# dimfeld/perceive

Hardware: AMD Instinct MI355X
Metric: vectors scanned/sec (exact cosine top-10, 384-d f32, batch=64) (higher is better)
Workload: dtype f32

## Files before the change

### perceive_amd/csrc/scan.h

```cpp
#pragma once
#include <hip/hip_runtime.h>
#include <stdint.h>

#include "../../include/perceive_hip.h"

namespace pcv {

constexpr int kBlockRows = 32;
constexpr int kMaxK = PCV_MAX_RESULTS;
constexpr int kSeedPartRows = 256;
constexpr int kSeedParts = 64;
constexpr int kMaxWaveQueries = 4;
constexpr int kHot = 256;
constexpr int kMfmaQueries = 256;
constexpr int kScale8Stride = 1;

struct SegDesc {
    const float4* blk;
    const float* scale;
    const int64_t* ids;
    int64_t id0;
    int64_t pos0;
    uint32_t nrows;
    uint32_t nblocks;
// ... 54 lines not shown

struct ScanParams {
    const SegDesc* seg;
    int nseg;
    uint32_t total_blocks;
    int D;
    int D4;
    int B;
    int k;
    int metric;
    uint32_t tile_rows;
    const CeilRec* ceil;
    const float* queries;
    float* qf32;
    uint16_t* qbf16;
    int8_t* q8;
    float* q8c;
    float* qraw;
    float* margin;
    float* margin32;
    uint32_t* tau;
    uint32_t* tau_c;
    uint32_t* slots;
    uint32_t* cand_cnt;
    uint64_t* cand;
    float* cand_s;
    pcv_hit_dev* out;
    pcv_hit_dev* out_host;
    uint32_t* cnt_host;
    uint32_t* coarse_host;
    pcv_hit_dev* flag_rec;
    uint32_t cand_cap;
    uint32_t seed_blocks;
    uint32_t seed_shift;
    uint32_t flags;
    unsigned long long* stamps;
    float eps16, eps32;
    float max_norm;
    uint32_t* spec;
    int spec_rank;
    float spec_gap;
    float spec_spread;
    float* spec_base_host;
    float* spec_top_host;
    float* kth_host;
    const RangeRec* range;
    pcv_hit_dev* range_out;
    uint32_t* range_cnt;
    uint32_t range_runs;
    uint32_t range_keep;
};
constexpr uint32_t kSpecFailed = 0xffffffffu;

struct DistinctRec {
    uint32_t kept, examined, flags, pad;
    double last_score;
    int64_t last_pos;
};
constexpr uint32_t kDistinctFull = 1u, kDistinctEnd = 2u;
struct DistinctArgs {
    DistinctRec* rec;
    DistinctRec* rec_host;
    pcv_hit_dev* kept;
    double* kept_norm;
    int32_t* similar;
    int num_results;
    double threshold;
};

struct GroupedArgs {
    DistinctRec* rec;
    DistinctRec* rec_host;
    pcv_hit_dev* kept;
    int64_t* kept_group;
// ... 29 lines not shown
    uint32_t u = (k & 0x80000000u) ? (k & 0x7fffffffu) : ~k;
    return __builtin_bit_cast(float, u);
}
constexpr uint32_t kKeyNegInf = 0x007fffffu;
__host__ __device__ static inline uint64_t f64_key(double d) {
    uint64_t u = __builtin_bit_cast(uint64_t, d);
    return (u >> 63) ? ~u : (u | 0x8000000000000000ull);
}
__host__ __device__ static inline double key_f64(uint64_t k) {
    uint64_t u = (k >> 63) ? (k & 0x7fffffffffffffffull) : ~k;
    return __builtin_bit_cast(double, u);
}

__host__ __device__ static inline float reported_score(int metric, int D, double c) {
    if (metric == PCV_METRIC_DOT) {
        const double d = 1.0 - c / (double)D;
        return (float)(d > 0.0 ? d : 0.0);
    }
    return (float)c;
}

void launch_upload(hipStream_t st, const void* src_pinned, void* dst, size_t bytes);
void launch_prep_seed(hipStream_t st, const ScanParams& p, const ScanParams* dp, const SegDesc& seg0);
void launch_scan_wave(hipStream_t st, const ScanParams& p, const ScanParams* dp, int num_cus);
void launch_scan_mfma(hipStream_t st, const ScanParams& p, const ScanParams* dp, int num_cus);
int mfma_pass_queries(int Dp);
uint32_t mfma_tile_rows(int B);
void launch_scan_mfma8(hipStream_t st, const ScanParams& p, const ScanParams* dp, int num_cus);
int mfma8_pass_queries(int Dp);
bool mfma8_six_pass(int B, int Dp, uint32_t flags, int nseg);
void launch_rescore_select(hipStream_t st, const ScanParams& p, const ScanParams* dp);
void launch_range_thresholds(hipStream_t st, const ScanParams& p, const ScanParams* dp);
void launch_range_select(hipStream_t st, const ScanParams& p, const ScanParams* dp);
void launch_distinct_select(hipStream_t st, const ScanParams& p, const ScanParams* dp, const DistinctArgs& a);
void launch_diverse_collect(hipStream_t st, const ScanParams& p, const ScanParams* dp, const DiverseArgs& a);
void launch_diverse_select(hipStream_t st, int B, int D, int D4, int metric, const DiverseArgs& a);
void launch_grouped_select(hipStream_t st, const ScanParams& p, const ScanParams* dp, const GroupedArgs& a);
void launch_reset_scan_state(hipStream_t st, uint32_t* tau, uint32_t* slots, uint32_t* cand_cnt);
void launch_merge(hipStream_t st, const pcv_hit_dev* lists, int n_shards, int B, int k, pcv_hit_dev* out,
                  int flagged = 0);
void launch_similarity_matrix(hipStream_t st, const float* a, int B, const float* m, int64_t N, int D, int cosine,
                              float* out);

}
```

### perceive_amd/csrc/scan_kernels.hip

```cpp
#include <algorithm>
#include <cassert>
#include <cstdlib>
#include <numeric>
#include <type_traits>

#include "common.h"
#include "device_access.h"
#include "scan.h"

namespace pcv {
namespace {

struct SegCursor {
    int si = -1;
    uint32_t begin = 0, end = 0;
    const float4* blk = nullptr;
    const float* scale = nullptr;
    const uint4* blk16 = nullptr;
    const uint4* blk8 = nullptr;
    const float* scale8 = nullptr;
    const uint4* mid16 = nullptr;
    const float* scale16 = nullptr;
    const uint4* blk6 = nullptr;
    const float4* scale6 = nullptr;
// ... 116 lines not shown
            }
            active = false;
        }
    }
}

__device__ __noinline__ void emit_hit(const ScanParams& p, int q, int seg, uint32_t row, float s,
                                      bool feeds_slots) {
    const int cc = ceil_class(p, q, s);
    if (cc == 2) return;
    feeds_slots = feeds_slots && cc == 0;
    uint32_t idx = g_atomic_add(&p.cand_cnt[q * kHot], 1u);
    if (idx < p.cand_cap) {
        gst(&p.cand[(size_t)q * p.cand_cap + idx], ((uint64_t)(uint32_t)seg << 32) | row);
        gst(&p.cand_s[(size_t)q * p.cand_cap + idx], s);
    }
    if (feeds_slots && isfinite(s)) offer_slot(p, q, s);
}


__global__ __launch_bounds__(256) void reset_scan_state_kernel(uint32_t* __restrict__ tau, uint32_t* __restrict__ slots,
                                                               uint32_t* __restrict__ cand_cnt) {
    const int t = blockIdx.x * 256 + threadIdx.x;
    if (t < kMfmaQueries * kMaxK) slots[t] = kKeyNegInf;
    if (t < kMfmaQueries) {
        tau[t * kHot] = kKeyNegInf;
        tau[kMfmaQueries * kHot + t] = kKeyNegInf;
        cand_cnt[t * kHot] = 0;
        cand_cnt[t * kHot + 32] = 0;
        cand_cnt[t * kHot + 33] = 0;
        cand_cnt[t * kHot + 34] = 0;
        cand_cnt[t * kHot + 35] = 0;
    }
}

__device__ __forceinline__ bool is_seed_block(const ScanParams& p, int si, uint32_t lb) {
    return si == 0 && (lb & ((1u << p.seed_shift) - 1u)) == 0 && (lb >> p.seed_shift) < p.seed_blocks;
}

__device__ __forceinline__ uint32_t seed_threshold_key(const ScanParams& p, int q, int sub ) {
    uint32_t mn = 0xffffffffu;
    if (q < p.B)
        for (int j = sub; j < p.k; j += 4) mn = min(mn, ld_relaxed(&p.slots[(size_t)q * kMaxK + j]));
    mn = min(mn, (uint32_t)__shfl_xor(mn, 1));
    mn = min(mn, (uint32_t)__shfl_xor(mn, 2));
    return q < p.B ? mn : kKeyNegInf;
}
// ... 100 lines not shown
#pragma unroll
        for (int j = 0; j < 16; ++j)
#pragma unroll
            for (int g = 0; g < QG; ++g) {
                const float4 qv = *(const float4*)&sq[g * Dp + (f0 + j) * 4];
                acc[g] = fmaf(qv.x, v[j].x, acc[g]);
                acc[g] = fmaf(qv.y, v[j].y, acc[g]);
                acc[g] = fmaf(qv.z, v[j].z, acc[g]);
                acc[g] = fmaf(qv.w, v[j].w, acc[g]);
            }
    }
    {
        const uint32_t grp = sr % (uint32_t)p.k;
#pragma unroll
        for (int g = 0; g < QG; ++g) {
            const float s = acc[g] * sc;
            if (sc != 0.0f && isfinite(s) && (q0 + g >= p.B || ceil_class(p, q0 + g, s) == 0)) atomicMax(&gmax[g * kMaxK + grp], f32_key(s));
        }
    }
    __syncthreads();
    for (int i = tid; i < QG * p.k; i += 256) {
        const int g = i / p.k, j = i - g * p.k, q = q0 + g;
        const uint32_t key = gmax[g * kMaxK + j];
        if (q < p.B && key != kKeyNegInf) g_atomic_max(&p.slots[(size_t)q * kMaxK + j], key);
    }
}

__global__ __launch_bounds__(256) void prep_seed_mfma_kernel(const ScanParams* __restrict__ pp, const float4* __restrict__ seg0_blk,
                                                             const float* __restrict__ seg0_scale, uint32_t nseed) {
    const ScanParams& p = *pp;
    extern __shared__ __attribute__((aligned(16))) float smem[];
    const int Dp = p.D4 * 4, D = p.D, LD = Dp + 4;
    float* sq = smem;
    uint32_t* gmax = (uint32_t*)(smem + 32 * LD);
    const int part = blockIdx.x, q0 = blockIdx.y * 32, tid = threadIdx.x, lane = tid & 63;
    const int wave = __builtin_amdgcn_readfirstlane(tid >> 6);
    const int r = lane & 31, h = lane >> 5;
    const bool writer = part == 0;
    const uint32_t sb = part * 4 + wave;
    const uint32_t lb = sb << p.seed_shift;
    const bool active = sb < p.seed_blocks && lb * 32u < nseed;
    const int P = p.D4 >> 1;
    const float4* base = seg0_blk + (size_t)(active ? lb : 0) * p.D4 * 32 + h * 32 + r;
    float4 va[16], vb[16];
    auto load16 = [&](float4 (&v)[16], int m0) {
#pragma unroll
        for (int j = 0; j < 16; ++j) v[j] = (active && m0 + j < P) ? gld4(base + (size_t)(m0 + j) * 64) : make_float4(0, 0, 0, 0);
// ... 41 lines not shown
            }
        }
        if (writer && have && sub == 0) {
            float unit = 1.0f;
            if (p.metric == PCV_METRIC_DOT) unit = (float)sqrt(sum) * p.max_norm * 1.0001f;
            gst(&p.margin[q], (p.eps16 + p.eps32) * unit);
            gst(&p.margin32[q], 2.0f * p.eps32 * unit);
        }
    }
    if (writer && blockIdx.y == 0) {
        uint16_t* z = p.qbf16 + (size_t)p.B * Dp;
        const int nz = ((int)p.tile_rows > p.B) ? ((int)p.tile_rows - p.B) * Dp : 0;
        for (int i = tid; i < nz; i += 256) gst(&z[i], (uint16_t)0);
        if (tid == 0 && p.flag_rec) {
            pcv_hit_dev f;
            f.score = 0.0;
            f.pos = 0;
            f.id = 0;
            *p.flag_rec = f;
        }
    }
    __syncthreads();

    f32x16 acc;
#pragma unroll
    for (int i = 0; i < 16; ++i) acc[i] = 0.0f;
    const float* qrow = sq + r * LD + h * 4;
    auto mma16 = [&](const float4 (&v)[16], int m0) {
#pragma unroll
        for (int j = 0; j < 16; ++j) {
            if (m0 + j < P) {
                const float4 qv = *(const float4*)&qrow[(m0 + j) * 8];
                acc = __builtin_amdgcn_mfma_f32_32x32x2f32(v[j].x, qv.x, acc, 0, 0, 0);
                acc = __builtin_amdgcn_mfma_f32_32x32x2f32(v[j].y, qv.y, acc, 0, 0, 0);
                acc = __builtin_amdgcn_mfma_f32_32x32x2f32(v[j].z, qv.z, acc, 0, 0, 0);
                acc = __builtin_amdgcn_mfma_f32_32x32x2f32(v[j].w, qv.w, acc, 0, 0, 0);
            }
        }
    };
    for (int m0 = 0; m0 < P; m0 += 32) {
        if (m0 + 16 < P) load16(vb, m0 + 16);
        __builtin_amdgcn_sched_barrier(0);
        mma16(va, m0);
        if (m0 + 32 < P) load16(va, m0 + 32);
        __builtin_amdgcn_sched_barrier(0);
        if (m0 + 16 < P) mma16(vb, m0 + 16);
    }
    if (active) {
        float sc[16];
#pragma unroll
        for (int i = 0; i < 16; ++i) {
            const uint32_t row = lb * 32 + (i & 3) + 8 * (i >> 2) + 4 * h;
            sc[i] = row < nseed ? gld(&seg0_scale[row]) : 0.0f;
        }
        const float clo = (p.ceil && q0 + r < p.B) ? gld(&p.ceil[q0 + r].lo) : __builtin_inff();
#pragma unroll
        for (int i = 0; i < 16; ++i) {
            const float s = acc[i] * sc[i];
            const uint32_t sr = sb * 32 + (i & 3) + 8 * (i >> 2) + 4 * h;
            if (sc[i] != 0.0f && isfinite(s) && s < clo) atomicMax(&gmax[r * p.k + sr % (uint32_t)p.k], f32_key(s));
        }
    }
    __syncthreads();
    for (int i = tid; i < 32 * p.k; i += 256) {
        const int g = i / p.k, j = i - g * p.k, q = q0 + g;
        const uint32_t key = gmax[i];
        if (q < p.B && key != kKeyNegInf) g_atomic_max(&p.slots[(size_t)q * kMaxK + j], key);
    }
}

struct BlockCursor {
    uint32_t gb;
    SegCursor sc;
    uint32_t lb;
    __amdgpu_buffer_rsrc_t rows;
    int ch;
};

template <int NB, bool NTL>
__global__ __launch_bounds__(256) void scan_wave_kernel(const ScanParams* __restrict__ pp) {
    const ScanParams& p = *pp;
    extern __shared__ __attribute__((aligned(16))) float sq[];
    const int Dp = p.D4 * 4;
    for (int i = threadIdx.x; i < NB * Dp; i += 256) sq[i] = gld(&p.qf32[i]);
    __syncthreads();
    const int lane = threadIdx.x & 63;
    const uint32_t wave = __builtin_amdgcn_readfirstlane(threadIdx.x >> 6);
    const int r = lane & 31, h = lane >> 5;
    float mrg[NB];
    uint32_t tau0[NB];
// ... 370 lines not shown
        for (int off = 32; off > 0; off >>= 1) {
            guess = max(guess, (uint32_t)__shfl_xor(guess, off));
            med = max(med, (uint32_t)__shfl_xor(med, off));
            top = max(top, (uint32_t)__shfl_xor(top, off));
        }
        if (learned && med != kKeyNegInf) {
            const float fm = key_f32(med), ft = key_f32(top);
            const float g = fminf(fm + p.spec_gap, ft + (ft - fm));
            const bool alike = fabsf((ft - fm) - p.spec_spread) <= 0.5f * p.spec_spread;
            if (alike && isfinite(g)) guess = max(guess, f32_key(g));
        }
        if (lane == 0 && guess != kKeyNegInf) {
            g_atomic_max(&p.tau[q * kHot], guess);
            g_atomic_max(&p.tau_c[q], guess);
        }
    }
    if (lane == 0 && have && p.spec_base_host) {
        p.spec_base_host[q] = med != kKeyNegInf ? key_f32(med) : __builtin_nanf("");
        p.spec_top_host[q] = top != kKeyNegInf ? key_f32(top) : __builtin_nanf("");
    }
    if (lane == 0) p.spec[q] = guess;
}

__global__ __launch_bounds__(256) void set_guess_kernel(const ScanParams* __restrict__ pp) {
    const ScanParams& p = *pp;
    const int q = blockIdx.x * 4 + (threadIdx.x >> 6);
    set_guess(p, q, threadIdx.x & 63, q < p.B);
}

__global__ __launch_bounds__(256) void quantize_queries_kernel(const ScanParams* __restrict__ pp) {
    const ScanParams& p = *pp;
    const int lane = threadIdx.x & 63;
    const int q = blockIdx.x * 4 + (threadIdx.x >> 6);
    const int Dp = p.D4 * 4, Dp8 = (Dp + 127) & ~127;
    const bool have = q < p.B;
    const float* src = p.qf32 + (size_t)q * Dp;
    float x[16];
    float mx = 0.0f, l1 = 0.0f;
#pragma unroll
    for (int j = 0; j < 16; ++j) {
        const int i = lane + 64 * j;
        x[j] = (have && i < Dp) ? gld(&src[i]) : 0.0f;
    }
#pragma unroll
    for (int j = 0; j < 16; ++j) {
        mx = fmaxf(mx, fabsf(x[j]));
        l1 += fabsf(x[j]);
    }
#pragma unroll
    for (int off = 32; off > 0; off >>= 1) {
        mx = fmaxf(mx, __shfl_xor(mx, off));
        l1 += __shfl_xor(l1, off);
    }
    const float s_q = (mx > 0.0f && mx < __builtin_inff() && l1 < __builtin_inff()) ? 127.0f / mx : 0.0f;
    int8_t* row = p.q8 + (size_t)q * Dp8;
    double n2 = 0.0, e2 = 0.0;
    int qs = 0, qa = 0;
#pragma unroll
    for (int j = 0; j < 16; ++j) {
        const int i = lane + 64 * j;
        const int qi = max(-127, min(127, (int)rintf((s_q != 0.0f ? x[j] : 0.0f) * s_q)));
        if (i < Dp8) row[i] = (int8_t)qi;
        const double e = s_q != 0.0f ? (double)x[j] - (double)qi / (double)s_q : 0.0;
        n2 += (double)x[j] * (double)x[j];
        e2 += e * e;
        qs += qi;
        qa += abs(qi);
    }
#pragma unroll
    for (int off = 32; off > 0; off >>= 1) {
        n2 += __shfl_xor(n2, off);
        e2 += __shfl_xor(e2, off);
        qs += __shfl_xor(qs, off);
        qa += __shfl_xor(qa, off);
    }
    if (lane == 0) {
        p.q8c[4 * q] = s_q;
        p.q8c[4 * q + 1] = 0.5002f * l1 * s_q + 0.2501f * (float)Dp8 + 4.0f;
        p.q8c[4 * q + 2] = l1;
        const bool live = have && s_q != 0.0f;
        const double W = 126.5 * (double)qs, M = 252.0 * (double)qa + fabs(W);
        const float up = 1.0f + 0x1p-19f;
        const float wn = (float)(-W + M * 0x1p-20);
        p.q8c[4 * kMfmaQueries + 4 * q] = live ? (float)(sqrt(n2) * (double)s_q) * up : 0.0f;
        p.q8c[4 * kMfmaQueries + 4 * q + 1] = live ? (float)(sqrt(e2) * (double)s_q) * up : 0.0f;
        p.q8c[4 * kMfmaQueries + 4 * q + 2] = live ? wn + fabsf(wn) * 0x1p-22f : 0.0f;
    }
    set_guess(p, q, lane, have);
}

template <int FROM, int TO, class F>
__device__ __forceinline__ bool static_for_until(F&& f) {
    if constexpr (FROM < TO) {
        if (f(std::integral_constant<int, FROM>{})) return true;
        return static_for_until<FROM + 1, TO>(f);
    } else {
        return false;
    }
}

constexpr uint32_t kRing = 2048;
constexpr int kRingSegBits = 18;
struct SurvRing {
    uint32_t lo[kRing], hi[kRing];
    int acc[kRing];
    float sblk[kRing];
    uint32_t tail, head, done, pad;
};
__device__ __forceinline__ uint32_t lds_ld(const uint32_t* p) { return __hip_atomic_load(p, __ATOMIC_RELAXED, __HIP_MEMORY_SCOPE_WORKGROUP); }
__device__ __forceinline__ void lds_st(uint32_t* p, uint32_t v) { __hip_atomic_store(p, v, __ATOMIC_RELAXED, __HIP_MEMORY_SCOPE_WORKGROUP); }
// ... 373 lines not shown
    __shared__ float lsq[NT * 32], lvq[NT * 32];
    __shared__ uint32_t ring_words[DRAIN ? sizeof(SurvRing) / 4 : 4];
    SurvRing& ring = *(SurvRing*)ring_words;
    __shared__ uint32_t stack_words[DRAIN ? sizeof(DrainStack) / 4 : 4];
    DrainStack& stack = *(DrainStack*)stack_words;
    __shared__ float lU[NT * 32];
    __shared__ float lT6[SIX ? NT * 32 : 1];
    const int lane = threadIdx.x & 63;
    const uint32_t wave = __builtin_amdgcn_readfirstlane(threadIdx.x >> 6);
    PCV_STAMP(0)
    if constexpr (DRAIN) {
        for (uint32_t i = threadIdx.x; i < kRing; i += WPB * 64) ring.hi[i] = 0u;
        if (threadIdx.x < 4) (&ring.tail)[threadIdx.x] = 0u;
    }
    for (int i = threadIdx.x; i < NT * 32 * P16; i += WPB * 64) {
        const int q = i / P16, pc = i - q * P16;
        lq8[(size_t)q * LDQ + pc] = __builtin_bit_cast(uint4, gld4((const float4*)p.q8 + i));
    }
    for (int q = threadIdx.x; q < NT * 32; q += WPB * 64) {
        lsq[q] = gld(&p.q8c[4 * q]);
        lvq[q] = gld(&p.q8c[4 * q + 1]);
    }
    for (int q = threadIdx.x >> 2; q < NT * 32; q += WPB * 16) {
        const uint32_t key = seed_threshold_key(p, q, threadIdx.x & 3);
        if ((threadIdx.x & 3) == 0) ltau0[q] = key;
    }
    __syncthreads();
    const int c = lane & 31, h = lane >> 5;
    const float nrm = (p.metric == PCV_METRIC_DOT) ? p.max_norm : 1.0f;
    const float c1 = 0.5002f * sqrtf((float)Dp8) * nrm;
    const float dead_u = (p.metric == PCV_METRIC_DOT) ? -__builtin_inff() : __builtin_inff();
    auto u_of = [&](int q, uint32_t tau_key, float e32q) -> float {
        const float sqq = lsq[q];
        const float T = (key_f32(max(ltau0[q], tau_key)) - e32q) * sqq;
        return (q < p.B) ? (sqq != 0.0f ? (T - fabsf(T) * 2e-6f) - c1 : dead_u) : __builtin_inff();
    };
    if constexpr (ULDS) {
        for (int q = threadIdx.x; q < NT * 32; q += WPB * 64) {
            const uint32_t tk = ld_relaxed(&p.tau_c[q]);
            const float e32q = q < p.B ? 0.5f * gld(&p.margin32[q]) : 0.0f;
            lU[q] = u_of(q, tk, e32q);
            if constexpr (SIX) {
                const float T = (key_f32(max(ltau0[q], tk)) - e32q) * lsq[q];
                lT6[q] = (q < p.B) ? (lsq[q] != 0.0f ? T - fabsf(T) * 2e-6f : dead_u) : __builtin_inff();
            }
        }
        __syncthreads();
// ... 294 lines not shown
template <bool NTL, int NCH, int NH>
__global__ __launch_bounds__(NH == 2 ? 256 : 768, 3) void scan_mfma8_hold_kernel(const ScanParams* __restrict__ pp) {
    const ScanParams& p = *pp;
    constexpr int TQ = NH * 64;
    constexpr int WPB = NH == 2 ? 4 : 12;
    extern __shared__ uint4 lq8[];
    constexpr int P16 = NCH * 8;
    constexpr int LDQ = P16 + 1;
    const int D4 = p.D4;
    __shared__ uint32_t ltau0[TQ];
    __shared__ float lsq[TQ], lvq[TQ], le32[TQ];
    const int lane = threadIdx.x & 63;
    const uint32_t wave = __builtin_amdgcn_readfirstlane(threadIdx.x >> 6);
    for (int i = threadIdx.x; i < TQ * P16; i += WPB * 64) {
        const int q = i / P16, pc = i - q * P16;
        lq8[(size_t)q * LDQ + pc] = __builtin_bit_cast(uint4, gld4((const float4*)p.q8 + i));
    }
    for (int q = threadIdx.x; q < TQ; q += WPB * 64) {
        lsq[q] = gld(&p.q8c[4 * q]);
        lvq[q] = gld(&p.q8c[4 * q + 1]);
        le32[q] = q < p.B ? 0.5f * gld(&p.margin32[q]) : 0.0f;
    }
    for (int q = threadIdx.x >> 2; q < TQ; q += WPB * 16) {
        const uint32_t key = seed_threshold_key(p, q, threadIdx.x & 3);
        if ((threadIdx.x & 3) == 0) ltau0[q] = key;
    }
    __syncthreads();
    const int c = lane & 31, h = lane >> 5;
    const float nrm = (p.metric == PCV_METRIC_DOT) ? p.max_norm : 1.0f;
    const float c1 = 0.5002f * sqrtf((float)(NCH * 128)) * nrm;
    const float dead = (p.metric == PCV_METRIC_DOT) ? -__builtin_inff() : __builtin_inff();
    __shared__ float lU[TQ];
    auto u_of = [&](int q, uint32_t tau_key) -> float {
        const float sq = lsq[q];
        const float T = (key_f32(max(ltau0[q], tau_key)) - le32[q]) * sq;
        const float live = (T - fabsf(T) * 2e-6f) - c1;
        return q < p.B ? (sq != 0.0f ? live : dead) : __builtin_inff();
    };
    for (int q = threadIdx.x; q < TQ; q += WPB * 64) lU[q] = u_of(q, ld_relaxed(&p.tau[q * kHot]));
    __syncthreads();

    const uint32_t total_waves = gridDim.x * WPB;
    struct Cur {
        uint32_t gb;
        SegCursor sc;
        uint32_t lb;
    } cur;
// ... 315 lines not shown
    }
    if (tid == 0 && nv < (uint32_t)p.k && p.kth_host) p.kth_host[q] = __builtin_nanf("");
    pcv_hit_dev none;
    none.score = __builtin_nan("");
    none.pos = -1;
    none.id = -1;
    for (int j = (int)nv + tid; j < p.k; j += 256) put(j, none);
    if (tid == 0) {
        const bool failed = guessed && n_spec < (uint32_t)p.k;
        if (p.cnt_host) p.cnt_host[q] = failed ? kSpecFailed : raw_cnt;
        if (p.coarse_host) {
            p.coarse_host[q] = ld_relaxed(&p.cand_cnt[q * kHot + 32]);
            p.coarse_host[kMfmaQueries + q] = ld_relaxed(&p.cand_cnt[q * kHot + 33]);
            p.coarse_host[2 * kMfmaQueries + q] = ld_relaxed(&p.cand_cnt[q * kHot + 34]);
        }
        st_relaxed(&p.cand_cnt[q * kHot + 32], 0u);
        st_relaxed(&p.cand_cnt[q * kHot + 33], 0u);
        st_relaxed(&p.cand_cnt[q * kHot + 34], 0u);
        if ((raw_cnt > p.cand_cap || failed) && p.flag_rec) p.flag_rec->pos = 1;
        st_relaxed(&p.tau[q * kHot], kKeyNegInf);
        st_relaxed(&p.tau_c[q], kKeyNegInf);
        st_relaxed(&p.cand_cnt[q * kHot], 0u);
    }
    for (int j = tid; j < p.k; j += 256) st_relaxed(&p.slots[(size_t)q * kMaxK + j], kKeyNegInf);
}

__global__ __launch_bounds__(kMfmaQueries) void range_thresholds_kernel(const ScanParams* __restrict__ pp) {
    const ScanParams& p = *pp;
    const int q = threadIdx.x;
    if (q >= p.B) return;
    const uint32_t key = f32_key(p.range[q].tau);
    st_relaxed(&p.tau[q * kHot], key);
    st_relaxed(&p.tau_c[q], key);
}

template <bool COOP>
__global__ __launch_bounds__(256) void range_select_kernel(const ScanParams* __restrict__ pp) {
    const ScanParams& p = *pp;
    extern __shared__ float4 lds4[];
    __shared__ uint32_t n_in, s_last;
    __shared__ double s_nq;
    const int q = blockIdx.y, tid = threadIdx.x;
    const uint32_t run = blockIdx.x;
    const int D4 = p.D4;
    float4* sq = lds4;
    float4* stage = lds4 + D4;
    double* c_s = (double*)(stage + (COOP ? 4 * 8 * (D4 + 1) : 0));
// ... 68 lines not shown
            hit.pos = c_p[r];
            hit.id = sg.ids ? sg.ids[row] : sg.id0 + (int64_t)row;
            out[r] = hit;
        }
    }
    if (tid == 0) p.range_cnt[(size_t)q * p.range_runs + run] = n;
    __syncthreads();
    if (tid == 0) s_last = g_atomic_add(&p.cand_cnt[q * kHot + 35], 1u) == gridDim.x - 1 ? 1u : 0u;
    __syncthreads();
    if (s_last && tid == 0) {
        if (p.cnt_host) p.cnt_host[q] = raw_cnt;
        if (p.coarse_host) {
            p.coarse_host[q] = ld_relaxed(&p.cand_cnt[q * kHot + 32]);
            p.coarse_host[kMfmaQueries + q] = ld_relaxed(&p.cand_cnt[q * kHot + 33]);
            p.coarse_host[2 * kMfmaQueries + q] = ld_relaxed(&p.cand_cnt[q * kHot + 34]);
        }
        st_relaxed(&p.cand_cnt[q * kHot + 32], 0u);
        st_relaxed(&p.cand_cnt[q * kHot + 33], 0u);
        st_relaxed(&p.cand_cnt[q * kHot + 34], 0u);
        st_relaxed(&p.cand_cnt[q * kHot + 35], 0u);
        st_relaxed(&p.tau[q * kHot], kKeyNegInf);
        st_relaxed(&p.tau_c[q], kKeyNegInf);
        st_relaxed(&p.cand_cnt[q * kHot], 0u);
        for (int j = 0; j < p.k; ++j) st_relaxed(&p.slots[(size_t)q * kMaxK + j], kKeyNegInf);
    }
}

__global__ __launch_bounds__(64) void merge_kernel(const pcv_hit_dev* __restrict__ lists_all, int n_shards, int B, int k,
                                                   size_t stride, int flagged, pcv_hit_dev* __restrict__ out) {
    extern __shared__ unsigned char taken[];
    const int q = blockIdx.x, lane = threadIdx.x;
    const int total = n_shards * k;
    if (flagged && q == 0 && lane == 0) {
        int64_t any = 0;
        for (int sh = 0; sh < n_shards; ++sh) any |= lists_all[sh * stride + (size_t)B * k].pos;
        pcv_hit_dev f;
        f.score = 0.0;
        f.pos = any ? 1 : 0;
        f.id = 0;
        out[(size_t)B * k] = f;
    }
    for (int i = lane; i < total; i += 64) taken[i] = 0;
    __syncthreads();
    for (int j = 0; j < k; ++j) {
        double bs = 0;
        int64_t bp = 0;
        int bi = -1;
// ... 45 lines not shown
    for (int i = 0; i < D; ++i) {
        dot = fmaf(q[i], x[i], dot);
        nq = fmaf(q[i], q[i], nq);
        nx = fmaf(x[i], x[i], nx);
    }
    out[(size_t)b * N + n] = cosine ? dot / (sqrtf(nq) * sqrtf(nx)) : dot;
}

}


void launch_reset_scan_state(hipStream_t st, uint32_t* tau, uint32_t* slots, uint32_t* cand_cnt) {
    reset_scan_state_kernel<<<kMfmaQueries * kMaxK / 256, 256, 0, st>>>(tau, slots, cand_cnt);
    PCV_LAUNCHED();
}

void launch_upload(hipStream_t st, const void* src_pinned, void* dst, size_t bytes) {
    const uint32_t n16 = (uint32_t)((bytes + 15) / 16);
    if (n16 == 0) return;
    upload_kernel<<<(n16 + 255) / 256, 256, 0, st>>>((const uint4*)src_pinned, (uint4*)dst, n16);
    PCV_LAUNCHED();
}

void launch_prep_seed(hipStream_t st, const ScanParams& p, const ScanParams* dp, const SegDesc& seg0) {
    const int nparts = std::max(1, (int)((p.seed_blocks * 32u + kSeedPartRows - 1) / kSeedPartRows));
    const uint32_t nseed = seg0.nrows;
    const size_t Dp = (size_t)p.D4 * 4;
    const size_t lds1 = Dp * sizeof(float) + kMaxK * sizeof(uint32_t);
    const size_t lds_mfma = 32 * (Dp + 4) * sizeof(float) + 32 * (size_t)p.k * sizeof(uint32_t);
    if (lds_mfma <= 156 * 1024 && !(p.flags & kFlagValuSeed)) {
        allow_dynamic_lds((const void*)prep_seed_mfma_kernel, lds_mfma);
        const unsigned parts = (p.seed_blocks + 3) / 4;
        prep_seed_mfma_kernel<<<dim3(parts ? parts : 1, (p.B + 31) / 32), 256, lds_mfma, st>>>(dp, seg0.blk, seg0.scale, nseed);
    } else if (p.B <= 2 || 8 * lds1 > 64 * 1024) {
        prep_seed_kernel<1><<<dim3(nparts, p.B), 256, lds1, st>>>(dp, seg0.blk, seg0.scale, nseed);
    } else if (p.B <= 32 || 16 * lds1 > 64 * 1024 || !(p.flags & kFlagSeed16)) {
        prep_seed_kernel<8><<<dim3(nparts, (p.B + 7) / 8), 256, 8 * lds1, st>>>(dp, seg0.blk, seg0.scale, nseed);
    } else {
        prep_seed_kernel<16><<<dim3(nparts, (p.B + 15) / 16), 256, 16 * lds1, st>>>(dp, seg0.blk, seg0.scale, nseed);
    }
    PCV_LAUNCHED();
}

void launch_scan_wave(hipStream_t st, const ScanParams& p, const ScanParams* dp, int num_cus) {
    if (p.total_blocks == 0) return;
    const size_t lds = (size_t)p.B * p.D4 * 4 * sizeof(float);
    const unsigned gm = flags_groups_per_cu(p.flags);
    unsigned grid = (unsigned)num_cus * (gm ? gm : 8);
    const unsigned need = (p.total_blocks + 3) / 4;
    if (grid > need) grid = need;
    const bool ntl = (p.flags & kFlagPlainLoads) == 0;
    for (const void* f : {(const void*)scan_wave_kernel<1, true>, (const void*)scan_wave_kernel<2, true>, (const void*)scan_wave_kernel<3, true>,
                          (const void*)scan_wave_kernel<4, true>, (const void*)scan_wave_kernel<1, false>, (const void*)scan_wave_kernel<2, false>,
                          (const void*)scan_wave_kernel<3, false>, (const void*)scan_wave_kernel<4, false>})
        allow_dynamic_lds(f, lds);
#define PCV_WAVE(NB)                                                   \
    if (ntl)                                                           \
        scan_wave_kernel<NB, true><<<grid, 256, lds, st>>>(dp);         \
    else                                                               \
        scan_wave_kernel<NB, false><<<grid, 256, lds, st>>>(dp);
    switch (p.B) {
        case 1: PCV_WAVE(1); break;
        case 2: PCV_WAVE(2); break;
        case 3: PCV_WAVE(3); break;
        default: PCV_WAVE(4); break;
    }
#undef PCV_WAVE
    PCV_LAUNCHED();
}

int mfma_pass_queries(int Dp) {
    for (int nt : {4, 2, 1})
        if ((size_t)nt * 32 * Dp * 2 <= 156 * 1024) return nt * 32;
    return 0;
}

uint32_t mfma_tile_rows(int B) { return B <= 32 ? 32u : (B <= 64 ? 64u : 128u); }

template <int NT, bool NTL, int WPB, int NBUF, bool SRC16>
static void launch_mfma_variant(hipStream_t st, const ScanParams* dp, unsigned grid, size_t lds) {
    allow_dynamic_lds((const void*)scan_mfma_kernel<NT, NTL, WPB, NBUF, SRC16>, lds);
    scan_mfma_kernel<NT, NTL, WPB, NBUF, SRC16><<<grid, WPB * 64, lds, st>>>(dp);
}

template <int NT, bool NTL>
static void launch_mfma_shape(hipStream_t st, const ScanParams* dp, unsigned grid, size_t lds, bool wide, bool src16, unsigned nbuf,
                              unsigned wpb) {
    if (src16) {
        if (NT == 4 || wide) {
            if (nbuf == 4) launch_mfma_variant<NT, NTL, 8, 4, true>(st, dp, grid, lds);
            else launch_mfma_variant<NT, NTL, 8, 6, true>(st, dp, grid, lds);
        } else if constexpr (NT < 4) {
            if (nbuf == 6) launch_mfma_variant<NT, NTL, 4, 6, true>(st, dp, grid, lds);
            else launch_mfma_variant<NT, NTL, 4, 4, true>(st, dp, grid, lds);
        }
        return;
    }
    if (NT == 4 || wide) launch_mfma_variant<NT, NTL, 8, 3, false>(st, dp, grid, lds);
    else if constexpr (NT < 4) launch_mfma_variant<NT, NTL, 4, 2, false>(st, dp, grid, lds);
}
// ... 53 lines not shown
static void launch_mfma8_six(hipStream_t st, const ScanParams* dp, unsigned grid, size_t lds, int nch) {
    switch (nch) {
        case 1: launch_mfma8_variant<NT, true, 12, kSixChunkBufs<NT>, true, 1, true>(st, dp, grid, lds); break;
        case 2: launch_mfma8_variant<NT, true, 12, kSixChunkBufs<NT>, true, 2, true>(st, dp, grid, lds); break;
        case 3: launch_mfma8_variant<NT, true, 12, kSixChunkBufs<NT>, true, 3, true>(st, dp, grid, lds); break;
        default: PCV_FAIL(PCV_ERR_INTERNAL, "6-bit screen: %d chunks per block", nch);
    }
}
template <int NT, bool NTL, int NBUF>
static void launch_mfma8_drain(hipStream_t st, const ScanParams* dp, unsigned grid, size_t lds, int nch) {
    switch (nch) {
        case 1: launch_mfma8_variant<NT, NTL, 12, NBUF, true, 1>(st, dp, grid, lds); break;
        case 2: launch_mfma8_variant<NT, NTL, 12, NBUF, true, 2>(st, dp, grid, lds); break;
        case 3: launch_mfma8_variant<NT, NTL, 12, NBUF, true, 3>(st, dp, grid, lds); break;
        case 4: launch_mfma8_variant<NT, NTL, 12, NBUF, true, 4>(st, dp, grid, lds); break;
        case 6: launch_mfma8_variant<NT, NTL, 12, NBUF, true, 6>(st, dp, grid, lds); break;
        case 8: launch_mfma8_variant<NT, NTL, 12, NBUF, true, 8>(st, dp, grid, lds); break;
        default: launch_mfma8_variant<NT, NTL, 12, NBUF, true, 0>(st, dp, grid, lds); break;
    }
}

void launch_scan_mfma8(hipStream_t st, const ScanParams& p, const ScanParams* dp, int num_cus) {
    if (p.total_blocks == 0) return;
    const int NT = p.B <= 32 ? 1 : (p.B <= 64 ? 2 : (p.B <= 128 ? 4 : 8));
    const size_t lds = mfma8_lds(NT, p.D4 * 4);
    const unsigned gm = flags_groups_per_cu(p.flags);
    const bool ntl = (p.flags & kFlagPlainLoads) == 0;
    const unsigned most = NT == 4 ? 2 : 3;
    const unsigned per_cu = (unsigned)std::max<size_t>(1, std::min<size_t>(most, (156 * 1024) / lds));
    const bool wide8 = NT == 4 && per_cu == 1;
    const unsigned wpbt = wide8 ? 8 : 4;
    unsigned grid = (unsigned)num_cus * (gm ? gm : per_cu);
    const unsigned need = (p.total_blocks + wpbt - 1) / wpbt;
    if (grid > need) grid = need;
    if (p.D4 * 4 > 1024) PCV_FAIL(PCV_ERR_UNSUPPORTED, "int8 screen: dimension %d is too large", p.D);
    quantize_queries_kernel<<<NT * 32 / 4, 256, 0, st>>>(dp);
    PCV_LAUNCHED();
    const int nch = ((p.D4 * 4 + 127) & ~127) >> 7;
    if (p.B > 64 && nch <= 3 && (p.B > 128 || !(p.flags & kFlagTile128))) {
        const bool four = p.B > 128;
        const size_t ldsh = mfma8_lds(four ? 8 : 4, p.D4 * 4) + (four && nch >= 2 ? 12 * 4096 : 0);
        const unsigned wpb = four ? 12 : 4;
        const unsigned g3 = std::min<unsigned>((unsigned)num_cus * (gm ? gm : (four ? 1u : 3u)), (p.total_blocks + wpb - 1) / wpb);
#define PCV_HOLD(NCHV, NHV)                                                                           \
    {                                                                                                 \
        allow_dynamic_lds(ntl ? (const void*)scan_mfma8_hold_kernel<true, NCHV, NHV> : (const void*)scan_mfma8_hold_kernel<false, NCHV, NHV>, ldsh); \
        if (ntl) scan_mfma8_hold_kernel<true, NCHV, NHV><<<g3, NHV == 2 ? 256 : 768, ldsh, st>>>(dp); \
        else scan_mfma8_hold_kernel<false, NCHV, NHV><<<g3, NHV == 2 ? 256 : 768, ldsh, st>>>(dp);    \
    }
        if (four) {
            if (nch == 3) PCV_HOLD(3, 4) else if (nch == 2) PCV_HOLD(2, 4) else PCV_HOLD(1, 4)
        } else {
            if (nch == 3) PCV_HOLD(3, 2) else if (nch == 2) PCV_HOLD(2, 2) else PCV_HOLD(1, 2)
        }
#undef PCV_HOLD
        PCV_LAUNCHED();
        return;
    }
    if (NT == 8) PCV_FAIL(PCV_ERR_UNSUPPORTED, "int8 screen: %d queries in one pass need rows of at most 384 features", p.B);
    if (NT <= 2 && p.B > 4 && !(p.flags & kFlagFourWave) && p.nseg < (1 << kRingSegBits) && lds + 68 * 1024 <= 156 * 1024) {
// ... 93 lines not shown
```

### perceive_amd/csrc/searcher_pass.cpp

```cpp
#include <chrono>
#include <cstdlib>
#include <cstring>

#include "searcher_pass.h"

namespace pcv {

void ensure_workspace(pcv_searcher* s) {
    const size_t Q = kMfmaQueries;
    s->d_qf32.ensure(Q * s->Dp);
    s->d_qraw.ensure(Q * s->Dp);
    s->d_qbf16.ensure(Q * s->Dp);
    s->d_q8.ensure(Q * (size_t)((s->Dp + 127) & ~127));
    s->d_q8c.ensure(Q * 8);
    s->d_spec.ensure(Q);
    s->d_margin.ensure(Q);
    s->d_margin32.ensure(Q);
    s->d_tau.ensure((Q + 1) * kHot);
    s->d_slots.ensure(Q * kMaxK);
    s->d_cnt.ensure(Q * kHot);
    s->d_cand.ensure(Q * s->cand_cap);
    s->d_cand_s.ensure(Q * s->cand_cap);
    s->d_hits.ensure(Q * kMaxK);
    s->pin.ensure(1);
    for (auto& e : s->ev)
        if (!e) PCV_HIP(hipEventCreate(&e));
}

namespace {

constexpr int64_t kGraphRows = (int64_t)4 << 20;

struct PassLayout {
    size_t off_seg, off_ceil, off_range, off_q, total;
};
PassLayout pass_layout(const pcv_searcher* s, size_t nseg, bool with_ceil) {
    PassLayout L;
    L.off_seg = align_up(sizeof(ScanParams));
    L.off_ceil = align_up(L.off_seg + nseg * sizeof(SegDesc));
    L.off_range = with_ceil ? align_up(L.off_ceil + (size_t)kMfmaQueries * sizeof(CeilRec)) : L.off_ceil;
    L.off_q = with_ceil ? align_up(L.off_range + (size_t)kMfmaQueries * sizeof(RangeRec)) : L.off_ceil;
    L.total = L.off_q + (size_t)kMfmaQueries * s->D * sizeof(float);
// ... 43 lines not shown
        have_mid = false;
    }
    PCV_REQUIRE(r.B <= 128 || (r.kernel == PCV_KERNEL_MFMA && src.src_kind == 2 && src_wanted == 2), "search: %d queries in one pass without int8 copies of every selected row", r.B);
    src.total_blocks = blk0;
    src.have_mid = have_mid && r.nseg > 0;
    src.flags = (s->scan_flags & ~kFlagsSearcherOwned) | (src.src_kind == 1 ? kFlagSrc16 : 0u) | (src.src_kind == 2 ? kFlagSrc8 : 0u);
    src.six = src.src_kind == 2 && have_six && r.nseg > 0 && s->kernel == PCV_KERNEL_AUTO && !(s->scan_flags & kTuneNoSix) &&
              mfma8_six_pass(r.B, s->Dp, src.flags, r.nseg);
    if (src.six) src.flags |= kFlagSix;
    return src;
}

void fill_params(pcv_searcher* s, const PassRequest& r, const PassLayout& L, const PassSource& src, ScanParams& p) {
    p = ScanParams{};
    p.seg = reinterpret_cast<const SegDesc*>(s->d_pass.p + L.off_seg);
    p.nseg = r.nseg;
    p.total_blocks = src.total_blocks;
    p.D = s->D;
    p.D4 = s->D4;
    p.B = r.B;
    p.k = r.k();
    p.metric = s->metric;
    p.tile_rows = r.kernel == PCV_KERNEL_MFMA ? mfma_tile_rows(r.B) : 0u;
    p.queries = reinterpret_cast<const float*>(s->d_pass.p + L.off_q);
    if (r.kind == PassRequest::kCeilings) {
        std::memcpy(s->pin_pass.p + L.off_ceil, r.topk.ceil, (size_t)r.B * sizeof(CeilRec));
        p.ceil = reinterpret_cast<const CeilRec*>(s->d_pass.p + L.off_ceil);
    }
    p.qf32 = s->d_qf32.p;
    p.qbf16 = s->d_qbf16.p;
    p.q8 = s->d_q8.p;
    p.q8c = s->d_q8c.p;
    p.qraw = s->d_qraw.p;
    p.margin = s->d_margin.p;
    p.margin32 = s->d_margin32.p;
    p.tau = s->d_tau.p;
    p.tau_c = s->d_tau.p + (size_t)kMfmaQueries * kHot;
    p.slots = s->d_slots.p;
    p.cand_cnt = s->d_cnt.p;
    p.cand = s->d_cand.p;
    p.cand_s = s->d_cand_s.p;
    p.cand_cap = s->cand_cap;
    p.out = s->d_hits.p;
    if (r.kind != PassRequest::kRange) {
        if (r.topk.d_out) p.out = r.topk.d_out;
        p.out_host = r.topk.download ? s->pin->hits : nullptr;
        p.flag_rec = r.topk.d_flag;
    }
    p.cnt_host = s->pin->cnt;
    p.coarse_host = s->pin->coarse;
    p.flags = src.flags;
    const uint32_t seed_parts = flags_seed_parts(s->scan_flags) ? flags_seed_parts(s->scan_flags) : kSeedParts;
    const uint32_t seg0_blocks = r.segs[0].g->nblocks();
    p.seed_blocks = std::min<uint32_t>(std::min<uint32_t>(seed_parts, kSeedParts) * kSeedPartRows / kBlockRows, seg0_blocks);
    p.seed_shift = 0;
    while (((uint64_t)p.seed_blocks << (p.seed_shift + 1)) <= seg0_blocks && p.seed_shift < 20) ++p.seed_shift;
    p.spec = s->d_spec.p;
    p.spec_rank = 0;
    p.spec_gap = NAN;
    p.spec_spread = 0.0f;
    p.spec_base_host = s->pin->spec_base;
// ... 447 lines not shown
```

Before: 21.69 billion.

## Fold int8 query quantization into seed kernel and compute guess in scan prologue

Moves per-query int8 quantization out of its own kernel and into extra blocks of the MFMA seed kernel. A second copy of the seed top-k slots (slots0) now lets the int8 scan prologue compute the speculative threshold guess itself, so the separate quantize/set_guess launches are no longer needed when k and B are small. This removes one or two serial kernel launches per pass. In exchange it adds duplicate atomics on the seed slots and makes the seed grid larger.

New measurement: 21.68 billion. About the same (-0.0%).

```diff
diff --git a/perceive_amd/csrc/scan.h b/perceive_amd/csrc/scan.h
--- a/perceive_amd/csrc/scan.h
+++ b/perceive_amd/csrc/scan.h
@@ -100,6 +100,8 @@
     uint32_t* tau;
     uint32_t* tau_c;
     uint32_t* slots;
+    uint32_t* slots0;
+    uint32_t q8_rows;
     uint32_t* cand_cnt;
     uint64_t* cand;
     float* cand_s;
@@ -128,6 +130,8 @@
     uint32_t range_runs;
     uint32_t range_keep;
 };
+constexpr int kPrologueGuessK = 16;
+constexpr bool prologue_guess(int k, int B) { return k <= kPrologueGuessK && B <= 128; }
 constexpr uint32_t kSpecFailed = 0xffffffffu;
 
 struct DistinctRec {
@@ -203,11 +207,13 @@
 
 void launch_upload(hipStream_t st, const void* src_pinned, void* dst, size_t bytes);
 void launch_prep_seed(hipStream_t st, const ScanParams& p, const ScanParams* dp, const SegDesc& seg0);
+bool seed_is_mfma(int Dp, int k, uint32_t flags);
 void launch_scan_wave(hipStream_t st, const ScanParams& p, const ScanParams* dp, int num_cus);
 void launch_scan_mfma(hipStream_t st, const ScanParams& p, const ScanParams* dp, int num_cus);
 int mfma_pass_queries(int Dp);
 uint32_t mfma_tile_rows(int B);
 void launch_scan_mfma8(hipStream_t st, const ScanParams& p, const ScanParams* dp, int num_cus);
+uint32_t mfma8_tile_rows(int B);
 int mfma8_pass_queries(int Dp);
 bool mfma8_six_pass(int B, int Dp, uint32_t flags, int nseg);
 void launch_rescore_select(hipStream_t st, const ScanParams& p, const ScanParams* dp);
diff --git a/perceive_amd/csrc/scan_kernels.hip b/perceive_amd/csrc/scan_kernels.hip
--- a/perceive_amd/csrc/scan_kernels.hip
+++ b/perceive_amd/csrc/scan_kernels.hip
@@ -162,7 +162,10 @@
 __global__ __launch_bounds__(256) void reset_scan_state_kernel(uint32_t* __restrict__ tau, uint32_t* __restrict__ slots,
                                                                uint32_t* __restrict__ cand_cnt) {
     const int t = blockIdx.x * 256 + threadIdx.x;
-    if (t < kMfmaQueries * kMaxK) slots[t] = kKeyNegInf;
+    if (t < kMfmaQueries * kMaxK) {
+        slots[t] = kKeyNegInf;
+        slots[kMfmaQueries * kMaxK + t] = kKeyNegInf;
+    }
     if (t < kMfmaQueries) {
         tau[t * kHot] = kKeyNegInf;
         tau[kMfmaQueries * kHot + t] = kKeyNegInf;
@@ -309,7 +312,67 @@
     for (int i = tid; i < QG * p.k; i += 256) {
         const int g = i / p.k, j = i - g * p.k, q = q0 + g;
         const uint32_t key = gmax[g * kMaxK + j];
-        if (q < p.B && key != kKeyNegInf) g_atomic_max(&p.slots[(size_t)q * kMaxK + j], key);
+        if (q < p.B && key != kKeyNegInf) {
+            g_atomic_max(&p.slots[(size_t)q * kMaxK + j], key);
+            g_atomic_max(&p.slots0[(size_t)q * kMaxK + j], key);
+        }
+    }
+}
+
+constexpr int kSeedQuantParts = 8;
+template <class Load>
+__device__ __forceinline__ void quantize_query(const ScanParams& p, int q, bool have, int lane, Load load) {
+    const int Dp = p.D4 * 4, Dp8 = (Dp + 127) & ~127;
+    float x[16];
+    float mx = 0.0f, l1 = 0.0f;
+#pragma unroll
+    for (int j = 0; j < 16; ++j) {
+        const int i = lane + 64 * j;
+        x[j] = (have && i < Dp) ? load(i) : 0.0f;
+    }
+#pragma unroll
+    for (int j = 0; j < 16; ++j) {
+        mx = fmaxf(mx, fabsf(x[j]));
+        l1 += fabsf(x[j]);
+    }
+#pragma unroll
+    for (int off = 32; off > 0; off >>= 1) {
+        mx = fmaxf(mx, __shfl_xor(mx, off));
+        l1 += __shfl_xor(l1, off);
+    }
+    const float s_q = (mx > 0.0f && mx < __builtin_inff() && l1 < __builtin_inff()) ? 127.0f / mx : 0.0f;
+    int8_t* row = p.q8 + (size_t)q * Dp8;
+    double n2 = 0.0, e2 = 0.0;
+    int qs = 0, qa = 0;
+#pragma unroll
+    for (int j = 0; j < 16; ++j) {
+        const int i = lane + 64 * j;
+        const int qi = max(-127, min(127, (int)rintf((s_q != 0.0f ? x[j] : 0.0f) * s_q)));
+        if (i < Dp8) row[i] = (int8_t)qi;
+        const double e = s_q != 0.0f ? (double)x[j] - (double)qi / (double)s_q : 0.0;
+        n2 += (double)x[j] * (double)x[j];
+        e2 += e * e;
+        qs += qi;
+        qa += abs(qi);
+    }
+#pragma unroll
+    for (int off = 32; off > 0; off >>= 1) {
+        n2 += __shfl_xor(n2, off);
+        e2 += __shfl_xor(e2, off);
+        qs += __shfl_xor(qs, off);
+        qa += __shfl_xor(qa, off);
+    }
+    if (lane == 0) {
+        p.q8c[4 * q] = s_q;
+        p.q8c[4 * q + 1] = 0.5002f * l1 * s_q + 0.2501f * (float)Dp8 + 4.0f;
+        p.q8c[4 * q + 2] = l1;
+        const bool live = have && s_q != 0.0f;
+        const double W = 126.5 * (double)qs, M = 252.0 * (double)qa + fabs(W);
+        const float up = 1.0f + 0x1p-19f;
+        const float wn = (float)(-W + M * 0x1p-20);
+        p.q8c[4 * kMfmaQueries + 4 * q] = live ? (float)(sqrt(n2) * (double)s_q) * up : 0.0f;
+        p.q8c[4 * kMfmaQueries + 4 * q + 1] = live ? (float)(sqrt(e2) * (double)s_q) * up : 0.0f;
+        p.q8c[4 * kMfmaQueries + 4 * q + 2] = live ? wn + fabsf(wn) * 0x1p-22f : 0.0f;
     }
 }
 
@@ -397,6 +460,20 @@
     }
     __syncthreads();
 
+    if (p.q8_rows) {
+        const int nparts = (int)gridDim.x - kSeedQuantParts;
+        if (part >= nparts) {
+            const int nq = (int)p.q8_rows >> 2;
+            const int qd_end = blockIdx.y == gridDim.y - 1 ? nq : min(nq, 8 * ((int)blockIdx.y + 1));
+            for (int qd = 8 * (int)blockIdx.y + (part - nparts); qd < qd_end; qd += kSeedQuantParts) {
+                const int q = 4 * qd + wave, g = q - q0;
+                const float* xrow = sq + (g < 32 ? g : 0) * LD;
+                quantize_query(p, q, q < p.B, lane, [&](int i) { return xrow[i]; });
+            }
+            return;
+        }
+    }
+
     f32x16 acc;
 #pragma unroll
     for (int i = 0; i < 16; ++i) acc[i] = 0.0f;
@@ -440,7 +517,10 @@
     for (int i = tid; i < 32 * p.k; i += 256) {
         const int g = i / p.k, j = i - g * p.k, q = q0 + g;
         const uint32_t key = gmax[i];
-        if (q < p.B && key != kKeyNegInf) g_atomic_max(&p.slots[(size_t)q * kMaxK + j], key);
+        if (q < p.B && key != kKeyNegInf) {
+            g_atomic_max(&p.slots[(size_t)q * kMaxK + j], key);
+            g_atomic_max(&p.slots0[(size_t)q * kMaxK + j], key);
+        }
     }
 }
 
@@ -857,6 +937,61 @@
     if (lane == 0) p.spec[q] = guess;
 }
 
+__device__ __forceinline__ uint32_t seed_guess_key(const ScanParams& p, int q, int sub, bool publish) {
+    const bool have = q < p.B;
+    const bool learned = p.spec_gap == p.spec_gap;
+    const uint32_t* sl = p.slots0 + (size_t)(have ? q : 0) * kMaxK;
+    uint32_t v[kPrologueGuessK];
+#pragma unroll
+    for (int i = 0; i < kPrologueGuessK; ++i) v[i] = (have && i < p.k) ? ld_relaxed(&sl[i]) : kKeyNegInf;
+    uint32_t mn = 0xffffffffu, top = kKeyNegInf;
+#pragma unroll
+    for (int i = 0; i < kPrologueGuessK; ++i) {
+        if (i < p.k) {
+            mn = min(mn, v[i]);
+            top = max(top, v[i]);
+        }
+    }
+    uint32_t guess = kKeyNegInf, med = kKeyNegInf;
+    const int mid = (p.k - 1) / 2;
+#pragma unroll
+    for (int j = 0; j < kPrologueGuessK / 4; ++j) {
+        const int a = sub + 4 * j;
+        const uint32_t va = sub == 0 ? v[4 * j] : (sub == 1 ? v[4 * j + 1] : (sub == 2 ? v[4 * j + 2] : v[4 * j + 3]));
+        int ahead = 0;
+#pragma unroll
+        for (int i = 0; i < kPrologueGuessK; ++i) ahead += (i < p.k && (v[i] > va || (v[i] == va && i < a))) ? 1 : 0;
+        if (a < p.k && ahead == p.spec_rank - 1) guess = va;
+        if (a < p.k && ahead == mid) med = va;
+    }
+    guess = max(guess, (uint32_t)__shfl_xor(guess, 1));
+    guess = max(guess, (uint32_t)__shfl_xor(guess, 2));
+    med = max(med, (uint32_t)__shfl_xor(med, 1));
+    med = max(med, (uint32_t)__shfl_xor(med, 2));
+    if (learned && med != kKeyNegInf) {
+        const float fm = key_f32(med), ft = key_f32(top);
+        const float g = fminf(fm + p.spec_gap, ft + (ft - fm));
+        const bool alike = fabsf((ft - fm) - p.spec_spread) <= 0.5f * p.spec_spread;
+        if (alike && isfinite(g)) guess = max(guess, f32_key(g));
+    }
+    if (publish && sub == 0 && have) {
+        if (guess != kKeyNegInf) {
+            g_atomic_max(&p.tau[q * kHot], guess);
+            g_atomic_max(&p.tau_c[q], guess);
+        }
+        if (p.spec_base_host) {
+            p.spec_base_host[q] = med != kKeyNegInf ? key_f32(med) : __builtin_nanf("");
+            p.spec_top_host[q] = top != kKeyNegInf ? key_f32(top) : __builtin_nanf("");
+        }
+        p.spec[q] = guess;
+    }
+    return have ? max(mn, guess) : kKeyNegInf;
+}
+__device__ __forceinline__ uint32_t prologue_key(const ScanParams& p, int q, int sub) {
+    const bool guessing = p.q8_rows != 0 && (p.spec_rank > 0 || p.spec_gap == p.spec_gap) && prologue_guess(p.k, p.B);
+    return guessing ? seed_guess_key(p, q, sub, blockIdx.x == 0) : seed_threshold_key(p, q, sub);
+}
+
 __global__ __launch_bounds__(256) void set_guess_kernel(const ScanParams* __restrict__ pp) {
     const ScanParams& p = *pp;
     const int q = blockIdx.x * 4 + (threadIdx.x >> 6);
@@ -867,60 +1002,9 @@
     const ScanParams& p = *pp;
     const int lane = threadIdx.x & 63;
     const int q = blockIdx.x * 4 + (threadIdx.x >> 6);
-    const int Dp = p.D4 * 4, Dp8 = (Dp + 127) & ~127;
     const bool have = q < p.B;
-    const float* src = p.qf32 + (size_t)q * Dp;
-    float x[16];
-    float mx = 0.0f, l1 = 0.0f;
-#pragma unroll
-    for (int j = 0; j < 16; ++j) {
-        const int i = lane + 64 * j;
-        x[j] = (have && i < Dp) ? gld(&src[i]) : 0.0f;
-    }
-#pragma unroll
-    for (int j = 0; j < 16; ++j) {
-        mx = fmaxf(mx, fabsf(x[j]));
-        l1 += fabsf(x[j]);
-    }
-#pragma unroll
-    for (int off = 32; off > 0; off >>= 1) {
-        mx = fmaxf(mx, __shfl_xor(mx, off));
-        l1 += __shfl_xor(l1, off);
-    }
-    const float s_q = (mx > 0.0f && mx < __builtin_inff() && l1 < __builtin_inff()) ? 127.0f / mx : 0.0f;
-    int8_t* row = p.q8 + (size_t)q * Dp8;
-    double n2 = 0.0, e2 = 0.0;
-    int qs = 0, qa = 0;
-#pragma unroll
-    for (int j = 0; j < 16; ++j) {
-        const int i = lane + 64 * j;
-        const int qi = max(-127, min(127, (int)rintf((s_q != 0.0f ? x[j] : 0.0f) * s_q)));
-        if (i < Dp8) row[i] = (int8_t)qi;
-        const double e = s_q != 0.0f ? (double)x[j] - (double)qi / (double)s_q : 0.0;
-        n2 += (double)x[j] * (double)x[j];
-        e2 += e * e;
-        qs += qi;
-        qa += abs(qi);
-    }
-#pragma unroll
-    for (int off = 32; off > 0; off >>= 1) {
-        n2 += __shfl_xor(n2, off);
-        e2 += __shfl_xor(e2, off);
-        qs += __shfl_xor(qs, off);
-        qa += __shfl_xor(qa, off);
-    }
-    if (lane == 0) {
-        p.q8c[4 * q] = s_q;
-        p.q8c[4 * q + 1] = 0.5002f * l1 * s_q + 0.2501f * (float)Dp8 + 4.0f;
-        p.q8c[4 * q + 2] = l1;
-        const bool live = have && s_q != 0.0f;
-        const double W = 126.5 * (double)qs, M = 252.0 * (double)qa + fabs(W);
-        const float up = 1.0f + 0x1p-19f;
-        const float wn = (float)(-W + M * 0x1p-20);
-        p.q8c[4 * kMfmaQueries + 4 * q] = live ? (float)(sqrt(n2) * (double)s_q) * up : 0.0f;
-        p.q8c[4 * kMfmaQueries + 4 * q + 1] = live ? (float)(sqrt(e2) * (double)s_q) * up : 0.0f;
-        p.q8c[4 * kMfmaQueries + 4 * q + 2] = live ? wn + fabsf(wn) * 0x1p-22f : 0.0f;
-    }
+    const float* src = p.qf32 + (size_t)q * (p.D4 * 4);
+    quantize_query(p, q, have, lane, [&](int i) { return gld(&src[i]); });
     set_guess(p, q, lane, have);
 }
 
@@ -1340,7 +1424,7 @@
         lvq[q] = gld(&p.q8c[4 * q + 1]);
     }
     for (int q = threadIdx.x >> 2; q < NT * 32; q += WPB * 16) {
-        const uint32_t key = seed_threshold_key(p, q, threadIdx.x & 3);
+        const uint32_t key = prologue_key(p, q, threadIdx.x & 3);
         if ((threadIdx.x & 3) == 0) ltau0[q] = key;
     }
     __syncthreads();
@@ -1681,7 +1765,7 @@
         le32[q] = q < p.B ? 0.5f * gld(&p.margin32[q]) : 0.0f;
     }
     for (int q = threadIdx.x >> 2; q < TQ; q += WPB * 16) {
-        const uint32_t key = seed_threshold_key(p, q, threadIdx.x & 3);
+        const uint32_t key = NH == 2 ? prologue_key(p, q, threadIdx.x & 3) : seed_threshold_key(p, q, threadIdx.x & 3);
         if ((threadIdx.x & 3) == 0) ltau0[q] = key;
     }
     __syncthreads();
@@ -2043,7 +2127,10 @@
         st_relaxed(&p.tau_c[q], kKeyNegInf);
         st_relaxed(&p.cand_cnt[q * kHot], 0u);
     }
-    for (int j = tid; j < p.k; j += 256) st_relaxed(&p.slots[(size_t)q * kMaxK + j], kKeyNegInf);
+    for (int j = tid; j < p.k; j += 256) {
+        st_relaxed(&p.slots[(size_t)q * kMaxK + j], kKeyNegInf);
+        st_relaxed(&p.slots0[(size_t)q * kMaxK + j], kKeyNegInf);
+    }
 }
 
 __global__ __launch_bounds__(kMfmaQueries) void range_thresholds_kernel(const ScanParams* __restrict__ pp) {
@@ -2158,7 +2245,10 @@
         st_relaxed(&p.tau[q * kHot], kKeyNegInf);
         st_relaxed(&p.tau_c[q], kKeyNegInf);
         st_relaxed(&p.cand_cnt[q * kHot], 0u);
-        for (int j = 0; j < p.k; ++j) st_relaxed(&p.slots[(size_t)q * kMaxK + j], kKeyNegInf);
+        for (int j = 0; j < p.k; ++j) {
+            st_relaxed(&p.slots[(size_t)q * kMaxK + j], kKeyNegInf);
+            st_relaxed(&p.slots0[(size_t)q * kMaxK + j], kKeyNegInf);
+        }
     }
 }
 
@@ -2250,16 +2340,19 @@
     PCV_LAUNCHED();
 }
 
+static size_t seed_mfma_lds(size_t Dp, int k) { return 32 * (Dp + 4) * sizeof(float) + 32 * (size_t)k * sizeof(uint32_t); }
+bool seed_is_mfma(int Dp, int k, uint32_t flags) { return seed_mfma_lds((size_t)Dp, k) <= 156 * 1024 && !(flags & kFlagValuSeed); }
 void launch_prep_seed(hipStream_t st, const ScanParams& p, const ScanParams* dp, const SegDesc& seg0) {
     const int nparts = std::max(1, (int)((p.seed_blocks * 32u + kSeedPartRows - 1) / kSeedPartRows));
     const uint32_t nseed = seg0.nrows;
     const size_t Dp = (size_t)p.D4 * 4;
     const size_t lds1 = Dp * sizeof(float) + kMaxK * sizeof(uint32_t);
-    const size_t lds_mfma = 32 * (Dp + 4) * sizeof(float) + 32 * (size_t)p.k * sizeof(uint32_t);
-    if (lds_mfma <= 156 * 1024 && !(p.flags & kFlagValuSeed)) {
+    const size_t lds_mfma = seed_mfma_lds(Dp, p.k);
+    PCV_REQUIRE(p.q8_rows == 0 || seed_is_mfma((int)Dp, p.k, p.flags), "int8 pass: the tile is left to a seed kernel that does not prepare it");
+    if (seed_is_mfma((int)Dp, p.k, p.flags)) {
         allow_dynamic_lds((const void*)prep_seed_mfma_kernel, lds_mfma);
         const unsigned parts = (p.seed_blocks + 3) / 4;
-        prep_seed_mfma_kernel<<<dim3(parts ? parts : 1, (p.B + 31) / 32), 256, lds_mfma, st>>>(dp, seg0.blk, seg0.scale, nseed);
+        prep_seed_mfma_kernel<<<dim3((parts ? parts : 1) + (p.q8_rows ? kSeedQuantParts : 0), (p.B + 31) / 32), 256, lds_mfma, st>>>(dp, seg0.blk, seg0.scale, nseed);
     } else if (p.B <= 2 || 8 * lds1 > 64 * 1024) {
         prep_seed_kernel<1><<<dim3(nparts, p.B), 256, lds1, st>>>(dp, seg0.blk, seg0.scale, nseed);
     } else if (p.B <= 32 || 16 * lds1 > 64 * 1024 || !(p.flags & kFlagSeed16)) {
@@ -2304,6 +2397,7 @@
 }
 
 uint32_t mfma_tile_rows(int B) { return B <= 32 ? 32u : (B <= 64 ? 64u : 128u); }
+uint32_t mfma8_tile_rows(int B) { return B <= 32 ? 32u : (B <= 64 ? 64u : (B <= 128 ? 128u : 256u)); }
 
 template <int NT, bool NTL, int WPB, int NBUF, bool SRC16>
 static void launch_mfma_variant(hipStream_t st, const ScanParams* dp, unsigned grid, size_t lds) {
@@ -2403,7 +2497,7 @@
 
 void launch_scan_mfma8(hipStream_t st, const ScanParams& p, const ScanParams* dp, int num_cus) {
     if (p.total_blocks == 0) return;
-    const int NT = p.B <= 32 ? 1 : (p.B <= 64 ? 2 : (p.B <= 128 ? 4 : 8));
+    const int NT = (int)mfma8_tile_rows(p.B) / 32;
     const size_t lds = mfma8_lds(NT, p.D4 * 4);
     const unsigned gm = flags_groups_per_cu(p.flags);
     const bool ntl = (p.flags & kFlagPlainLoads) == 0;
@@ -2415,8 +2509,13 @@
     const unsigned need = (p.total_blocks + wpbt - 1) / wpbt;
     if (grid > need) grid = need;
     if (p.D4 * 4 > 1024) PCV_FAIL(PCV_ERR_UNSUPPORTED, "int8 screen: dimension %d is too large", p.D);
-    quantize_queries_kernel<<<NT * 32 / 4, 256, 0, st>>>(dp);
-    PCV_LAUNCHED();
+    if (!p.q8_rows) {
+        quantize_queries_kernel<<<NT * 32 / 4, 256, 0, st>>>(dp);
+        PCV_LAUNCHED();
+    } else if ((p.spec_rank > 0 || p.spec_gap == p.spec_gap) && !prologue_guess(p.k, p.B)) {
+        set_guess_kernel<<<(p.B + 3) / 4, 256, 0, st>>>(dp);
+        PCV_LAUNCHED();
+    }
     const int nch = ((p.D4 * 4 + 127) & ~127) >> 7;
     if (p.B > 64 && nch <= 3 && (p.B > 128 || !(p.flags & kFlagTile128))) {
         const bool four = p.B > 128;
diff --git a/perceive_amd/csrc/searcher_pass.cpp b/perceive_amd/csrc/searcher_pass.cpp
--- a/perceive_amd/csrc/searcher_pass.cpp
+++ b/perceive_amd/csrc/searcher_pass.cpp
@@ -17,7 +17,7 @@
     s->d_margin.ensure(Q);
     s->d_margin32.ensure(Q);
     s->d_tau.ensure((Q + 1) * kHot);
-    s->d_slots.ensure(Q * kMaxK);
+    s->d_slots.ensure(2 * Q * kMaxK);
     s->d_cnt.ensure(Q * kHot);
     s->d_cand.ensure(Q * s->cand_cap);
     s->d_cand_s.ensure(Q * s->cand_cap);
@@ -107,6 +107,7 @@
     p.k = r.k();
     p.metric = s->metric;
     p.tile_rows = r.kernel == PCV_KERNEL_MFMA ? mfma_tile_rows(r.B) : 0u;
+    p.q8_rows = (src.src_kind == 2 && seed_is_mfma(s->Dp, r.k(), src.flags)) ? mfma8_tile_rows(r.B) : 0u;
     p.queries = reinterpret_cast<const float*>(s->d_pass.p + L.off_q);
     if (r.kind == PassRequest::kCeilings) {
         std::memcpy(s->pin_pass.p + L.off_ceil, r.topk.ceil, (size_t)r.B * sizeof(CeilRec));
@@ -122,6 +123,7 @@
     p.tau = s->d_tau.p;
     p.tau_c = s->d_tau.p + (size_t)kMfmaQueries * kHot;
     p.slots = s->d_slots.p;
+    p.slots0 = s->d_slots.p + (size_t)kMfmaQueries * kMaxK;
     p.cand_cnt = s->d_cnt.p;
     p.cand = s->d_cand.p;
     p.cand_s = s->d_cand_s.p;
```
